# DanieleTeni/Online-Non-Linear-Centroidal-MPC-with-stability-Guarantees-for-Robust-Locomotion-of-Legged-Robots-

Measured on AMD Instinct MI355X. Metric: centroidal-MPC solves/sec, N=20 horizon, higher is better.
Workload: dtype f64

## Files before the change

### __graft_entry__.py

```python
import os
import sys

ROOT = os.path.dirname(os.path.abspath(__file__))
if ROOT not in sys.path:
    sys.path.insert(0, ROOT)


def build():
    import build as _b
    _b.build_hip()
    _b.build_oracle()
    _b.build_emu()
    _b.build_emu_gain()
    _b.build_emu_consts()
    _b.build_device_unit()
    _b.build_tools()
    import ctypes
    import torch
    import cmpc_amd
    from cmpc_amd import capi
    lib = ctypes.CDLL(capi.LIB_PATH)
    for sym in capi.SYMBOLS:
        getattr(lib, sym)


def smoke():
    import numpy as np
    import torch
    import cmpc_amd
    from cmpc_amd import workloads as wl
    from cmpc_amd.solver import BatchedCentroidalMPC
    from oracle import oracle_lib as ol

    assert torch.cuda.is_available(), "smoke() needs a GPU"
    spec, rec = wl.make_workload("perturbed", B=8, N=10, scale=0.25)
    solver = BatchedCentroidalMPC(spec, device="cuda:0")
    out, status, iters, kkt = solver.solve(torch.from_numpy(rec).to("cuda:0"))
# ... 18 lines not shown
```

### build.py

```python
import os
import subprocess
import sys

ROOT = os.path.dirname(os.path.abspath(__file__))
PKG = os.path.join(ROOT, "online-non-linear-centroidal-mpc-with-stability-guarantees-for-robust-locomotion-of-legged-robots-_amd")


def _newer(target, sources):
    if not os.path.exists(target):
        return True
    t = os.path.getmtime(target)
    return any(os.path.getmtime(s) > t for s in sources)


def build_hip(force=False, verbose=False):
    src = os.path.join(PKG, "csrc", "cmpc_hip.hip")
    wbc = os.path.join(PKG, "csrc", "wbc_qp.hip")
    deps = [src, wbc, os.path.join(PKG, "csrc", "cmpc_kernel.hpp"), os.path.join(PKG, "csrc", "cmpc_lds_asm.hpp"), os.path.join(PKG, "csrc", "cmpc_wave.hpp"), os.path.join(PKG, "csrc", "cmpc_order_fit.h"),
            os.path.join(ROOT, "include", "cmpc.h"), os.path.join(ROOT, "include", "cmpc_wbc.h")]
    out = os.path.join(PKG, "libcmpc_amd.so")
    if force or _newer(out, deps):
        cmd = ["hipcc", "--offload-arch=gfx950", "-O3", "-std=c++17", "-fPIC", "-shared", "-o", out, src, wbc]
        if verbose:
            cmd.insert(1, "-Rpass-analysis=kernel-resource-usage")
# ... 44 lines not shown

def build_emu_gain(force=False):
    src = os.path.join(ROOT, "tests", "emu", "cmpc_emu_gain.cpp")
    out = os.path.join(ROOT, "tests", "emu", "libcmpc_emu_gain.so")
    deps = [src, os.path.join(ROOT, "tests", "emu", "cmpc_emu.cpp"), os.path.join(PKG, "csrc", "cmpc_kernel.hpp"),
            os.path.join(PKG, "csrc", "cmpc_lds_asm.hpp"), os.path.join(PKG, "csrc", "cmpc_wave.hpp"),
            os.path.join(ROOT, "include", "cmpc.h")]
    if force or _newer(out, deps):
        subprocess.check_call(["g++", "-O2", "-std=c++17", "-mfma", "-ffp-contract=off", "-fPIC", "-shared", "-pthread", "-o", out, src])
    return out


def build_emu_consts(force=False):
    src = os.path.join(ROOT, "tests", "emu", "cmpc_emu_consts.cpp")
    out = os.path.join(ROOT, "tests", "emu", "libcmpc_emu_consts.so")
    deps = [src, os.path.join(ROOT, "tests", "emu", "cmpc_emu.cpp"), os.path.join(PKG, "csrc", "cmpc_kernel.hpp"),
            os.path.join(PKG, "csrc", "cmpc_lds_asm.hpp"), os.path.join(PKG, "csrc", "cmpc_wave.hpp"),
            os.path.join(ROOT, "include", "cmpc.h")]
    if force or _newer(out, deps):
        subprocess.check_call(["g++", "-O2", "-std=c++17", "-mfma", "-ffp-contract=off", "-fPIC", "-shared", "-pthread", "-o", out, src])
    return out


def build_device_unit(force=False):
    src = os.path.join(ROOT, "tests", "gpu_unit", "cmpc_device_unit.hip")
    out = os.path.join(ROOT, "tests", "gpu_unit", "libcmpc_device_unit.so")
    deps = [src, os.path.join(PKG, "csrc", "cmpc_kernel.hpp"), os.path.join(PKG, "csrc", "cmpc_lds_asm.hpp"), os.path.join(PKG, "csrc", "cmpc_wave.hpp")]
    if force or _newer(out, deps):
        subprocess.check_call(["hipcc", "--offload-arch=gfx950", "-O3", "-std=c++17", "-fPIC", "-shared", "-o", out, src])
    return out


def build_tools(force=False):
    outs = []
    for name in ("hbm_calib", "lds_b128_repro"):
        src = os.path.join(ROOT, "tools", "ubench", name + ".hip")
        out = os.path.join(ROOT, "tools", "ubench", name)
        if force or _newer(out, [src]):
            r = subprocess.run(["hipcc", "--offload-arch=gfx950", "-O3", "-o", out, src], capture_output=True, text=True)
            if r.returncode != 0:
                print(f"build_tools: {name} failed to compile (profiling scripts that need it will not run)\n{r.stderr}",
                      file=sys.stderr)
                continue
        outs.append(out)
    return outs


if __name__ == "__main__":
    force = "--force" in sys.argv
    print(build_hip(force, verbose="-v" in sys.argv))
    print(build_oracle(force))
    print(build_emu(force))
    print(build_emu_gain(force))
    print(build_emu_consts(force))
    print(build_device_unit(force))
    print(build_tools(force))
```

### online-non-linear-centroidal-mpc-with-stability-guarantees-for-robust-locomotion-of-legged-robots-_amd/csrc/cmpc_hip.hip

```cpp
#include <hip/hip_runtime.h>
#include <stdio.h>
#include <stdlib.h>
#include <string.h>
#include <string>

#include "cmpc_kernel.hpp"
#include "cmpc_order_fit.h"

#ifndef CMPC_WAVES_PER_SIMD
#define CMPC_WAVES_PER_SIMD 2
#endif

namespace {

constexpr int ORDER_BUCKETS = 64;
constexpr int ORDER_COUNTERS = 3 + 2 * ORDER_BUCKETS;

__device__ __forceinline__ int cmpc_order_bucket(const double *__restrict__ r, int N, double omega, double cz_max) {
  double gl = r[24 + 17], gr = r[24 + 18];
  const double gl0 = gl, gr0 = gr;
  int first = N, nsw = 0;
  double gain = 0.0;
  for (int k = 1; k <= N; ++k) {
    const double l = (k < N) ? r[24 + 19 * k + 17] : r[22], q = (k < N) ? r[24 + 19 * k + 18] : r[23];
// ... 391 lines not shown
  h->grid = h->num_cu * resident_per_cu(spec->nv);
  if (spec->nv == 4) {
    h->pair_per_cu = pairs_per_cu();
#ifdef CMPC_DEV_KNOBS
    if (const char *e = getenv("CMPC_PAIR_PER_CU")) { if (atoi(e) == 2 && h->pair_per_cu > 2) h->pair_per_cu = 2; }
#endif
    h->pair_grid = h->num_cu * h->pair_per_cu;
    h->pair_max_batch = (h->pair_per_cu >= 3 ? 14 : 8) * h->num_cu;
    if (spec->kernel == CMPC_KERNEL_SINGLE) h->pair_max_batch = 0;
    if (spec->kernel == CMPC_KERNEL_PAIR) h->pair_max_batch = 1 << 30;
#ifdef CMPC_DEV_KNOBS
    if (const char *e = getenv("CMPC_PAIR")) h->pair_max_batch = (atoi(e) == 0) ? 0 : 1 << 30;
#endif
  }
  h->slabs = slab_count(spec, h->num_cu);
#ifdef CMPC_DEV_KNOBS
  if (const char *e = getenv("CMPC_WG_PER_CU")) {
    const int n = atoi(e);
    if (n >= 1 && n < resident_per_cu(spec->nv)) h->grid = h->num_cu * n;
  }
#endif
  h->slab_doubles = slab_doubles(spec);
#ifdef CMPC_PROFILE
  if (hipMalloc(&h->prof, 28 * sizeof(long long)) == hipSuccess) (void)hipMemset(h->prof, 0, 28 * sizeof(long long));
#endif
  if (hipMalloc(&h->scratch, (size_t)h->slabs * h->slab_doubles * sizeof(double)) != hipSuccess ||
      hipMalloc(&h->ticket, ORDER_COUNTERS * sizeof(int)) != hipSuccess || hipEventCreate(&h->ev0) != hipSuccess ||
      hipEventCreate(&h->ev1) != hipSuccess) {
    cmpc_destroy(h);
    return fail(nullptr, "cmpc_create: device allocation failed");
  }
  *out = h;
  return 0;
}

int cmpc_destroy(cmpc_handle *h) {
  if (!h) return 0;
  DeviceGuard guard(h->device);
  if (h->scratch) (void)hipFree(h->scratch);
  if (h->ticket) (void)hipFree(h->ticket);
  if (h->order) (void)hipFree(h->order);
  if (h->gbuf) (void)hipFree(h->gbuf);
  if (h->ev0) (void)hipEventDestroy(h->ev0);
  if (h->ev1) (void)hipEventDestroy(h->ev1);
  delete h;
  return 0;
}
// ... 204 lines not shown
  const int blocks = B < 256 * 32 ? B : 256 * 32;
  hipLaunchKernelGGL(cmpc_build_records_kernel, dim3((unsigned)blocks), dim3(256), 0, (hipStream_t)stream, tb->T, N, rate,
                     B, nrec, t, state, tb->com_tab, tb->pose_l, tb->pose_r, tb->gl, tb->gr, tb->cur_l, tb->cur_r,
                     plan_pos, tb->n_steps, tb->slot_l, tb->slot_r, records);
  if (hipGetLastError() != hipSuccess) return fail(nullptr, "cmpc_build_records: launch failed");
  return 0;
}

const char *cmpc_last_kernel_name(cmpc_handle *h) { return h ? h->last_kernel : ""; }
const char *cmpc_last_error(cmpc_handle *h) { return h ? h->err.c_str() : g_err.c_str(); }
const char *cmpc_version(void) { return "cmpc_amd 0.5 (gfx950)"; }

#ifdef CMPC_DEV_KNOBS
int cmpc_debug_slab(cmpc_handle *h, double **ptr, size_t *doubles) {
  if (!h || !ptr || !doubles) return 1;
  *ptr = h->scratch; *doubles = h->slab_doubles;
  return 0;
}
#endif

#ifdef CMPC_PROFILE
int cmpc_profile_read(cmpc_handle *h, long long *out8) {
  if (!h || !h->prof) return 1;
  if (hipMemcpy(out8, h->prof, 28 * sizeof(long long), hipMemcpyDeviceToHost) != hipSuccess) return 1;
  (void)hipMemset(h->prof, 0, 28 * sizeof(long long));
  return 0;
}
#endif

}
```

### online-non-linear-centroidal-mpc-with-stability-guarantees-for-robust-locomotion-of-legged-robots-_amd/csrc/cmpc_kernel.hpp

```cpp
#pragma once
#include "../../include/cmpc.h"
#include <math.h>
#include <utility>
#ifdef CMPC_HOST_EMU
#include <cstdio>
#include <cstdlib>
#endif

#ifndef CMPC_HOST_EMU
#include <hip/hip_runtime.h>
#define CMPC_DEV __device__ __forceinline__
#define CMPC_LANE ((int)threadIdx.x)
#define CMPC_SYNC() asm volatile("s_waitcnt lgkmcnt(0)" ::: "memory")
#define CMPC_SYNC_GLOBAL() __syncthreads()
#define CMPC_SYNC_WG() asm volatile("s_waitcnt lgkmcnt(0)\n\ts_barrier" ::: "memory")
#define CMPC_WAVE_ID() ((int)__builtin_amdgcn_readfirstlane((int)threadIdx.x >> 6))
static __device__ __forceinline__ double cmpc_bcast(double v, int src) {
  union { double d; int i[2]; } u; u.d = v;
  u.i[0] = __builtin_amdgcn_readlane(u.i[0], src);
  u.i[1] = __builtin_amdgcn_readlane(u.i[1], src);
  return u.d;
}
#define CMPC_BCAST(v, src) cmpc_bcast((v), (src))
typedef double cmpc_v4d __attribute__((ext_vector_type(4)));
#define CMPC_MFMA_F64(a, b, c) __builtin_amdgcn_mfma_f64_16x16x4f64((a), (b), (c), 0, 0, 0)
#include "cmpc_wave.hpp"
#define CMPC_PAIR_OF(M, v, a, b) cmpc_pair_of<M>((v), (a), (b))
#define CMPC_OPAQUE(x) asm volatile("" : "+v"(x))
#define CMPC_OPAQUE_D(x) asm volatile("" : "+v"(x))
#define CMPC_UNIFORM_INT(x) __builtin_amdgcn_readfirstlane(x)
static __device__ __forceinline__ double cmpc_fresh(double a) { asm volatile("" : "+s"(a)); return a; }
#define CMPC_FRESH_D(x) cmpc_fresh(x)
#ifdef CMPC_FRESH_SPEC
#define SPD(field) cmpc_fresh(CMPC_SPEC_OR_ROW(field))
#else
#define SPD(field) CMPC_SPEC_OR_ROW(field)
#endif
typedef const double __attribute__((address_space(4))) *cmpc_crow_t;
#define CMPC_CROW(p) ((cmpc_crow_t)(p))
static __device__ __forceinline__ cmpc_crow_t cmpc_fresh_row(cmpc_crow_t r) { asm volatile("" : "+s"(r)); return r; }
#define CMPC_ROW_AT(r, i) (cmpc_fresh_row(r)[i])
static __device__ __forceinline__ double cmpc_uniform_d(double v) {
  union { double d; int i[2]; } u; u.d = v;
  int lo, hi;
  asm("s_nop 0\n\tv_readfirstlane_b32 %0, %2\n\tv_readfirstlane_b32 %1, %3\n\ts_nop 1" : "=s"(lo), "=s"(hi) : "v"(u.i[0]), "v"(u.i[1]));
  u.i[0] = lo; u.i[1] = hi;
  return u.d;
}
#ifdef CMPC_NO_UNIFORM_D
#define CMPC_UNIFORM_D(x) (x)
#else
#define CMPC_UNIFORM_D(x) cmpc_uniform_d(x)
#endif
#define CMPC_SCHED_FENCE() __builtin_amdgcn_sched_barrier(0)
#define CMPC_RELANE(x) do { (x) = (int)__builtin_amdgcn_mbcnt_hi(~0u, __builtin_amdgcn_mbcnt_lo(~0u, 0u)) + lane_base; } while (0)
#define CMPC_SYNC_WAVE(w) CMPC_SYNC()
#define CMPC_FENCE_WAVE(w) asm volatile("s_waitcnt vmcnt(0) lgkmcnt(0)" ::: "memory")
#endif
#ifdef CMPC_HOST_EMU
// ... 1 lines not shown
#define CMPC_FENCE_WAVE(w) emu_barrier_wait(&emu_wave_barrier[(w)])
#define CMPC_SYNC_WG() emu_barrier_wait(&emu_barrier)
#endif
#ifndef CMPC_RELANE
#define CMPC_RELANE(x) do { } while (0)
#define SPD(field) CMPC_SPEC_OR_ROW(field)
typedef const double *cmpc_crow_t;
#define CMPC_CROW(p) ((cmpc_crow_t)(p))
#define CMPC_ROW_AT(r, i) ((r)[i])
#define CMPC_FRESH_D(x) (x)
#define CMPC_UNIFORM_D(x) (x)
#endif
#define CMPC_CIDX(field) ((int)((__builtin_offsetof(cmpc_spec, field) - __builtin_offsetof(cmpc_spec, delta)) / sizeof(double)))
#define CMPC_SPEC_OR_ROW(field) (CONSTS ? CMPC_ROW_AT(crow, CMPC_CIDX(field)) : sp.field)
static_assert(CMPC_CIDX(relax) == CMPC_NCONST - 1 && CMPC_CIDX(box[2]) == 13 && __builtin_offsetof(cmpc_spec, tol) == __builtin_offsetof(cmpc_spec, relax) + sizeof(double),
              "the row of per-instance constants is the block of cmpc_spec from delta to relax");
#define CMPC_FMA(x, y, z) __builtin_fma((x), (y), (z))
#ifndef CMPC_OPAQUE_D
#define CMPC_OPAQUE_D(x) do { } while (0)
#endif
#ifndef CMPC_UNIFORM_INT
#define CMPC_UNIFORM_INT(x) (x)
#endif

#if defined(CMPC_PROFILE) && !defined(CMPC_HOST_EMU)
#define CMPC_TICK(slot) do { long long now_ = clock64(); tprof[slot] += now_ - tlast; tlast = now_; } while (0)
#define CMPC_TICK_RESET() do { tlast = clock64(); } while (0)
#else
#define CMPC_TICK(slot) do { } while (0)
#define CMPC_TICK_RESET() do { } while (0)
#endif

namespace cmpc {

struct KArgs {
  cmpc_spec sp;
  int B;
  const double *recs;
  const double *warm;
  const double *state_in;
  double *state_out;
  double *out;
  int32_t *status;
  int32_t *iters;
  double *kkt;
  double *scratch;
  size_t scratch_stride;
  long long *prof;
  double tol_acc, tol_tenth;
};

enum { R_LYAP = 0, R_CZ = 1, R_HWC = 2, R_BOX = 3, R_FRIC = 15 };

constexpr double ACC_FACTOR = 100.0;
// ... 154 lines not shown
  static_assert(3 * S::NF <= S::NZ, "r_j fits");
  static constexpr int LDS_DOUBLES = oEND + (oEND & 1);
};

template <int NV, int NW = 1, bool PIPE = false> struct Dims : LdsMap<NV, NW, PIPE> {
  using S = Sizes<NV, NW>;
  using Lm = LdsMap<NV, NW, PIPE>;
  static constexpr int WS = S::WS, NF = S::NF, NU = S::NU, NXA = S::NXA, NZ = S::NZ, NI = S::NI, NTRI = S::NTRI, NH = S::NH,
                       PS = S::PS, LS = S::LS, NPT = S::NPT;
  static constexpr bool COMPACT = (NV == 4 && NW == 1);
  static constexpr int gM = 0;
  static constexpr bool W_MERGE = (NZ <= WS);
  static constexpr int gAL = ((NTRI + 7) / 8) * 8;
  static constexpr int gGH = gAL + NZ;
  static constexpr int GHS = WS * NH;
  static constexpr int gB = gGH + 3 * GHS;
  static constexpr int gPB = gB + NXA;
  static constexpr int gPV = gPB + NXA;
  static constexpr int gL = gPV + NXA;
  static constexpr int gG = gL + NU;
  static constexpr int gL1 = gG + NI;
  static constexpr int gPV1 = gL1 + NU;
  static constexpr int STAGE = ((gPV1 + NXA + 7) / 8) * 8;
  static constexpr int state_lam(int N) { return CMPC_NSOL(N, NV); }
  static constexpr int state_s(int N) { return state_lam(N) + (N + 1) * NXA; }
  static constexpr int state_z(int N) { return state_s(N) + (N + 1) * NI; }
  static constexpr int state_mu(int N) { return state_z(N) + (N + 1) * NI; }
  static constexpr int state_fl(int N) { return state_mu(N) + 8; }
  static_assert(state_fl(20) + 2 * 21 == CMPC_NSTATE(20, NV), "layout of include/cmpc.h");
  static size_t scratch_doubles(int N) {
    size_t n = (size_t)(N + 1) * STAGE;
    n += (size_t)(N + 1) * NXA * 4;
    n += (size_t)(N + 1) * NU * 3;
    n += (size_t)(N + 1) * NI * 4;
    return (n + 7) / 8 * 8;
  }
};

#ifndef CMPC_NO_DEVICE_CODE

CMPC_DEV int tri(int i) { return i * (i + 1) / 2; }

typedef double cmpc_v2d __attribute__((vector_size(16)));
struct GArr {
  double *p;
  CMPC_DEV double &operator[](unsigned i) const { return *(double *)((char *)p + (size_t)(i * 8u)); }
  CMPC_DEV cmpc_v2d &pair(unsigned i) const { return *(cmpc_v2d *)((char *)p + (size_t)(i * 16u)); }
};

CMPC_DEV bool consts_row_ok(cmpc_crow_t row) {
  bool ok = true;
  for (int i = 0; i < CMPC_NCONST; ++i) {
    const double v = row[i];
    const bool positive = i == CMPC_CIDX(delta) || i == CMPC_CIDX(g) || (i >= CMPC_CIDX(cz_max) && i <= CMPC_CIDX(foot_width));
    const bool gain = i == CMPC_CIDX(k1) || i == CMPC_CIDX(k2);
    ok = ok && v < INFINITY && v > -INFINITY && (positive ? v > 0.0 : (gain || v >= 0.0));
  }
  return ok;
}

template <int NV, int NW = 1, bool PIPE = false, bool GAIN = false, bool CONSTS = false> struct Solver {
  using D = Dims<NV, NW, PIPE>;
  static constexpr int XCH_DU = 16, XCH_DOUBLES = XCH_DU + 2 * D::NU;
  static_assert(!PIPE || XCH_DOUBLES <= D::P_DOUBLES, "the exchange words fit in the unused P region of the second image");
  static constexpr int XCH_AT = D::LDS_DOUBLES + D::oP;
  static_assert(!PIPE || NW == 1, "the pipelined pair runs the one-wave solver");
  static_assert(!PIPE || (D::oUB + 64 <= D::oBV && D::oUB >= D::oXN1 + D::NXA && !D::GT_FIRST),
                "pair_vectors reads BV / writes XN1 of the image the Riccati wave is working in");
  static constexpr int NF = D::NF, NU = D::NU, NXA = D::NXA, NZ = D::NZ, NI = D::NI, NH = D::NH, WS = D::WS;
  static_assert(NW == 1 || NU <= 64, "the input rows (pivot chains, substitutions) live in the first wave");

  const KArgs &ka;
  const cmpc_spec &sp;
  double *lds;
  double *ldsR;
  int lane_base = 0;
  GArr gs;
  GArr rec;
  int N, lane;
  int wv = 0;
  GArr gx, glam, gdx, glamn, gu, gdu, gupx, gsl, gz, gds, gdz;
  int lr[NH][6];
  double lg[NH][6];
  double piv_min = PIV_MIN;
  GArr st_in{nullptr};
  long long tprof[28] = {0, 0, 0, 0, 0, 0, 0, 0, 0, 0, 0, 0, 0, 0, 0, 0, 0, 0, 0, 0, 0, 0, 0, 0, 0, 0, 0, 0}, tlast = 0;
  double *gain_out = nullptr;
  GArr gbuf{nullptr};
  bool gain_sweep = false;
  cmpc_crow_t crow = nullptr;

  CMPC_DEV Solver(const KArgs &a, double *l, double *g, const double *r)
      : ka(a), sp(a.sp), lds(l), ldsR(l), gs{g}, rec{const_cast<double *>(r)}, N(a.sp.N), lane(CMPC_LANE) {
    if constexpr (NW > 1 || PIPE) wv = CMPC_WAVE_ID();
    if constexpr (NW > 1) lane_base = 64 * wv;
    if constexpr (PIPE) lane &= 63;
    if constexpr (NW == 1 && !PIPE) CMPC_RELANE(lane);
    double *p = g + (size_t)(N + 1) * D::STAGE;
    gx = GArr{p}; p += (size_t)(N + 1) * NXA;
    glam = GArr{p}; p += (size_t)(N + 1) * NXA;
    gdx = GArr{p}; p += (size_t)(N + 1) * NXA;
    glamn = GArr{p}; p += (size_t)(N + 1) * NXA;
    gu = GArr{p}; p += (size_t)(N + 1) * NU;
    gdu = GArr{p}; p += (size_t)(N + 1) * NU;
    gupx = GArr{p}; p += (size_t)(N + 1) * NU;
    gsl = GArr{p}; p += (size_t)(N + 1) * NI;
    gz = GArr{p}; p += (size_t)(N + 1) * NI;
    gds = GArr{p}; p += (size_t)(N + 1) * NI;
    gdz = GArr{p};
  }
  CMPC_DEV GArr stage(int k) const { return GArr{gs.p + (size_t)k * D::STAGE}; }
  CMPC_DEV double &L(int o) const { return lds[o]; }
  CMPC_DEV double &R(int o) const { return ldsR[o]; }
  CMPC_DEV void image(int k) { if constexpr (PIPE) lds = ldsR + (k & 1) * D::LDS_DOUBLES; }
  CMPC_DEV void sync() const {
    if constexpr (PIPE) { CMPC_SYNC_WAVE(wv); }
    else {
#ifdef CMPC_HOST_EMU
      CMPC_SYNC();
#else
      if constexpr (NW == 1) CMPC_SYNC(); else CMPC_SYNC_WG();
#endif
    }
  }
  CMPC_DEV void gsync() const {
    if constexpr (PIPE) { CMPC_FENCE_WAVE(wv); } else { CMPC_SYNC_GLOBAL(); }
  }
  CMPC_DEV void pair_sync() const { if constexpr (PIPE) { CMPC_SYNC_GLOBAL(); } }
  CMPC_DEV bool first_wave() const { return NW == 1 || wv == 0; }

  CMPC_DEV double gam_k(int k, int f) const { return (k == N) ? L(D::oHDR + 22 + f) : L(D::oSR + 17 + f); }
  CMPC_DEV double gam_km1(int f) const { return L(D::oSRP + 17 + f); }
  CMPC_DEV void vert_local(int j, double &vx, double &vy) const {
    const double Lh = SPD(foot_length) * 0.5, Wh = SPD(foot_width) * 0.5;
// ... 944 lines not shown
        for (int q = 0; q < NXA; q += 4) {
          b0 += pr[q] * bv[q]; b1 += pr[q + 1] * bv[q + 1]; b2 += pr[q + 2] * bv[q + 2]; b3 += pr[q + 3] * bv[q + 3];
        }
      } else {
        const double *pr = &R(D::oP + lane * D::PS);
#pragma unroll
        for (int q = 0; q < NXA; q += 4) {
          b0 += pr[q] * bv[q]; b1 += pr[q + 1] * bv[q + 1]; b2 += pr[q + 2] * bv[q + 2]; b3 += pr[q + 3] * bv[q + 3];
        }
      }
      const double a = (b0 + b1) + (b2 + b3);
      L(D::oXN1 + lane) = R(D::oPC + lane) + a;
      st[D::gB + lane] = L(D::oBV + lane);
    }
  }
  CMPC_DEV double list_dot(int h, const double *v) const {
    double a = 0.0;
#pragma unroll
    for (int n = 0; n < 6; ++n) a = CMPC_FMA(lg[h][n], v[lr[h][n]], a);
    CMPC_OPAQUE_D(a);
    return a;
  }

  CMPC_DEV void eval_stage(int k, double mu, double reg, double wz, double x0n2, Err &er, bool init) {
    CMPC_RELANE(lane); CMPC_OPAQUE(lane);
    load_stage(k);
    CMPC_TICK(24);
    const GArr st = stage(k);
    if (k < N) {
      stage_geometry(k);
    } else {
      for (int c = lane; c < 3 * NZ; c += WS) L(D::oGH + c) = 0.0;
      if (lane < NXA) L(D::oBV + lane) = 0.0;
      sync();
    }
    CMPC_TICK(11);
    double gl_dot[NH];
    if constexpr (D::GT_FIRST) {
      if (k < N && lane < NXA) er.e_p = fmax(er.e_p, fabs(L(D::oBV + lane)));
      build_list(&L(D::oGH), (k < N) ? L(D::oSR + 17) : 0.0, (k < N) ? L(D::oSR + 18) : 0.0, L(D::oHDR + 20));
      if (lane < NZ) { st[D::gGH + lane] = lg[0][1]; st[D::gGH + D::GHS + lane] = lg[0][2]; st[D::gGH + 2 * D::GHS + lane] = lg[0][3]; }
      if (k < N) {
        form_Pb(st);
        sync();
        CMPC_TICK(13);
        gl_dot[0] = list_dot(0, &L(D::oLAMN));
        if (lane < NZ) { L(D::oH0 + lane) = list_dot(0, &L(D::oXN1)); L(D::oH1 + lane) = list_dot(0, &R(D::oPC1)); }
        gt_phase<false>(L(D::oSR + 17), L(D::oSR + 18), L(D::oHDR + 20));
      } else {
        gl_dot[0] = 0.0;
        for (int e = lane; e < D::NTRI; e += WS) L(D::oM + e) = 0.0;
        sync();
      }
      CMPC_RELANE(lane); CMPC_OPAQUE(lane);
    }
    stage_ineq(k, x0n2);
    CMPC_TICK(12);
    for (int r = lane; r < NI; r += WS) {
      const bool act = L(D::oW2 + r) != 0.0;
      const double g = L(D::oGK + r);
      double s = L(D::oSK + r), z = L(D::oZK + r);
      if (init) {
        const bool carry = act && s > 0.0 && z > 0.0;
        s = carry ? s : (act ? fmax(-g, fmin(1e-2, sqrt(mu))) : 1.0);
        z = carry ? z : (act ? mu / s : 0.0);
        L(D::oZK + r) = z;
        gsl[k * NI + r] = s; gz[k * NI + r] = z;
      }
      if (act) {
        double sg = z / s;
        if constexpr (GAIN) { if (gain_sweep) sg = fmin(sg, (r >= R_BOX && r < R_FRIC) ? GAIN_SIG_CAP_BOX : GAIN_SIG_CAP); }
        L(D::oW0 + r) = sg; L(D::oW1 + r) = sg * (g + s); L(D::oW2 + r) = 1.0 / s;
        er.e_p = fmax(er.e_p, fabs(g + s));
        er.e_c = fmax(er.e_c, fabs(s * z)); er.e_cmu = fmax(er.e_cmu, fabs(s * z - mu));
        er.sum_mult += fabs(z); er.n_mult += 1;
      } else {
        L(D::oW0 + r) = 0.0; L(D::oW1 + r) = 0.0; L(D::oW2 + r) = 0.0; L(D::oZK + r) = 0.0;
      }
// ... 9 lines not shown
      CMPC_RELANE(lane); CMPC_OPAQUE(lane);
      build_list(&L(D::oGH), (k < N) ? L(D::oSR + 17) : 0.0, (k < N) ? L(D::oSR + 18) : 0.0, L(D::oHDR + 20));
    }
#pragma unroll
    for (int h = 0; h < NH; ++h) {
      const int col = lane + WS * h;
      if (col >= NZ) continue;
      const double ho = cost_grad(k, col, wz);
      double jw[3];
      jgt3(k, col, jw);
      double r = ho + jw[0];
      if constexpr (D::GT) {
        if constexpr (!D::GT_FIRST) gl_dot[h] = (k < N) ? list_dot(h, &L(D::oLAMN)) : 0.0;
        r += gl_dot[h];
      } else {
        if (k < N) for (int n = 0; n < 6; ++n) r += lg[h][n] * L(D::oLAMN + lr[h][n]);
      }
      if (col >= NU) r -= L(D::oLAMK + col - NU);
      const bool is_var = (col < NU) ? (k < N) : (k >= 1);
      if (is_var) er.e_d = fmax(er.e_d, fabs(r));
      double h0 = ho + jw[1] + mu * jw[2];
      double h1 = jw[2];
      CMPC_OPAQUE_D(h0); CMPC_OPAQUE_D(h1);
      if constexpr (D::GT_FIRST) {
        if (k < N) { L(D::oH0 + col) = h0 + L(D::oH0 + col); L(D::oH1 + col) = h1 + L(D::oH1 + col); }
        else { L(D::oH0 + col) = h0; L(D::oH1 + col) = h1; }
      } else {
        L(D::oH0 + col) = h0; L(D::oH1 + col) = h1;
      }
      st[D::gAL + col] = L(D::oAL + col);
    }
    CMPC_TICK(26);
    if constexpr (!D::GT_FIRST) {
#pragma unroll
      for (int h = 0; h < NH; ++h) {
        const int c = lane + WS * h;
        if (c < NZ) { st[D::gGH + c] = L(D::oGH + c); st[D::gGH + D::GHS + c] = L(D::oGH + NZ + c); st[D::gGH + 2 * D::GHS + c] = L(D::oGH + 2 * NZ + c); }
      }
    }
    for (int r = lane; r < NI; r += WS) st[D::gG + r] = L(D::oGK + r);
    CMPC_TICK(0);
    if constexpr (D::GT_FIRST) {
      CMPC_RELANE(lane); CMPC_OPAQUE(lane);
      build_H(k, reg, wz);
      CMPC_TICK(1);
    }
    sync();
  }
  CMPC_DEV bool riccati_stage(int k) {
    const GArr st = stage(k);
    if constexpr (PIPE) {
      CMPC_RELANE(lane); CMPC_OPAQUE(lane);
      build_list(&L(D::oGH), (k < N) ? L(D::oSR + 17) : 0.0, (k < N) ? L(D::oSR + 18) : 0.0, L(D::oHDR + 20));
    }
    if (k < N) {
      if constexpr (!D::GT_FIRST) {
        if constexpr (!PIPE) form_Pb(st);
        sync();
        CMPC_TICK(13);
        CMPC_RELANE(lane); CMPC_OPAQUE(lane);
        gt_phase<true>(L(D::oSR + 17), L(D::oSR + 18), L(D::oHDR + 20));
        CMPC_TICK(14);
      }
      CMPC_RELANE(lane); CMPC_OPAQUE(lane);
// ... 48 lines not shown
            cmpc_lds_word pa[14];
            double v[14];
#pragma unroll
            for (int q = 0; q < 14; ++q) {
              const cmpc_lds_word alt = wc + CMPC_LDS_WORDS(tri(NU + q0 + q) + NU - (q0 + q));
              pa[q] = (wt > alt) ? wt : alt;
            }
            if (q0 == 0) lds_read_gather_off14<0>(v, pa); else lds_read_gather_off14<14>(v, pa);
#pragma unroll
            for (int q = 0; q < 14; ++q) pr[q0 + q] = v[q];
          }
        }
#pragma unroll
        for (int q = 0; q < NXA; q += 4) {
          b0 += pr[q] * bv[q]; b1 += pr[q + 1] * bv[q + 1]; b2 += pr[q + 2] * bv[q + 2]; b3 += pr[q + 3] * bv[q + 3];
        }
        other[D::oXN1 + lane] = (b0 + b1) + (b2 + b3);
        stage(k - 1)[D::gB + lane] = bv[lane];
      }
    }
    sync();
  }

  CMPC_DEV bool matrix_sweep(double mu, double reg, double x0n2, Err &er, bool init) {
    er.e_d = er.e_p = er.e_c = er.e_cmu = er.sum_mult = 0.0; er.n_mult = 0;
    piv_min = fmax(PIV_MIN, PIV_FRAC * reg);
    const double e1 = 2.718281828459045235360287;
    double ez = CMPC_UNIFORM_D(exp(-(double)(N - 1)));
    CMPC_OPAQUE_D(ez);
    if constexpr (!PIPE) {
      for (int k = N; k >= 0; --k) {
        const double wz = SPD(w_cz_const) * 0.5 * ez + SPD(w_cz_const) * 0.5;
        ez *= e1;
        eval_stage(k, mu, reg, wz, x0n2, er, init);
        if (!riccati_stage(k)) return false;
      }
      return true;
    } else {
      double *xch = ldsR + XCH_AT;
      if (lane == 0 && wv == 0) { xch[8] = 0.0; xch[9] = 0.0; }
      CMPC_SYNC_WG();
      for (int j = 0; j <= N + 2; ++j) {
        if (wv == 1) {
          const int kv = N - j + 2, k = N - j;
          if (kv >= 0 && kv <= N) { image(kv); pair_vectors(kv); }
          const double wz = SPD(w_cz_const) * 0.5 * ez + SPD(w_cz_const) * 0.5;
          ez *= e1;
          if (k >= 0) { image(k); eval_stage(k, mu, reg, wz, x0n2, er, init); }
        } else if (j >= 1 && j <= N + 1) {
          const int k = N - j + 1;
          image(k);
          if (!riccati_stage(k) && lane == 0) xch[8 + (j & 1)] = 1.0;
        }
        CMPC_SYNC_WG();
        const bool failed = xch[8 + (j & 1)] != 0.0;
        if (failed) { image(0); CMPC_SYNC_WG(); return false; }
      }
      image(0);
// ... 550 lines not shown
        for (int c = 0; c < G; ++c) { const double du = CMPC_BCAST(y[c], cu); acc[c] += cf * du; }
      } else {
        const int sx = col - NU;
        if (sx < G) acc[sx] += cf;
      }
    }
    if (lane < CMPC_NX) {
#pragma unroll
      for (int c = 0; c < G; ++c) gout[lane * G + c] = acc[c];
    }
  }

  CMPC_DEV void gain_tail(int st, bool saved, const double *warm) {
    const bool usable = st == CMPC_CONVERGED || st == CMPC_ACCEPTABLE;
    bool good = false;
    if (usable) {
      if (saved) {
        st_in = gbuf;
        if (!PIPE || wv == 0) initial_point(gbuf.p, warm, true);
        if constexpr (PIPE) pair_sync(); else gsync();
      }
      Err er;
      gain_sweep = true;
      good = matrix_sweep(sp.tol, 0.0, 0.0, er, false);
      if constexpr (PIPE) pair_sync(); else gsync();
    }
    if (wv == 0) gain_step(good);
    if constexpr (PIPE) pair_sync(); else gsync();
  }

  CMPC_DEV void reject(double *state_out, double *out_, int32_t *status, int32_t *iters, double *kkt_out) {
    if (!PIPE || wv == 0) {
      const GArr out{out_};
      const double nanv = __builtin_nan("");
      for (int e = lane; e < (N + 1) * CMPC_NX + N * NU; e += WS) out[e] = nanv;
      if (lane == 0) {
        *status = CMPC_NUMERICAL; *iters = 0; *kkt_out = INFINITY;
        if (state_out) { GArr{state_out}[D::state_mu(N)] = 0.0; GArr{state_out}[D::state_mu(N) + 1] = 0.0; }
      }
    }
    if constexpr (PIPE) pair_sync(); else sync();
  }

  CMPC_DEV void solve(const double *warm, const double *state_in, double *state_out, double *out, int32_t *status,
                      int32_t *iters, double *kkt_out) {
    auto tol_ = [&]() { return CMPC_FRESH_D(sp.tol); };
    const double tol_acc = ka.tol_acc, tol_10 = ka.tol_tenth;
    const double x0n2 = 0.0;
    bool resume = false;
    if (state_in) {
      const double ms = GArr{const_cast<double *>(state_in)}[D::state_mu(N)];
      resume = ms > 0.0 && ms < INFINITY;
      if (resume) st_in = GArr{const_cast<double *>(state_in)};
    }
    int st = CMPC_MAX_ITER, it = 0, spent = 0;
    bool ret_saved = false;
    double kkt = INFINITY;
    for (;;) {
    if (state_out && lane == 0) GArr{state_out}[D::state_mu(N)] = 0.0;
    double mu = resume ? st_in[D::state_mu(N)] : MU_INIT;
    kkt = INFINITY; st = CMPC_MAX_ITER;
    constexpr bool CNT_LDS = (NW == 1);
    int n_acc = 0, n_stall = 0, polish = -1, since_best = 0;
    constexpr int SAVED = 256;
    constexpr int NOSTEP = 512;
    double &reg_last = R(D::oCOLD + 0), &kkt_best = R(D::oCOLD + 1), &kkt_saved = R(D::oCOLD + 2);
    double &snapped = R(D::oCOLD + 3);
    {
      double inf = INFINITY, zero = 0.0;
      CMPC_OPAQUE_D(inf); CMPC_OPAQUE_D(zero);
      const double ks0 = kkt_saved;
      if constexpr (PIPE) { CMPC_SYNC_WG(); } else sync();
      double at0 = sp.acc_tol;
      CMPC_OPAQUE_D(at0);
      const bool carry = spent > 0 && ks0 <= fmax(at0, tol_());
      reg_last = zero; kkt_best = inf; snapped = zero;
      if (!carry) kkt_saved = inf;
      if constexpr (CNT_LDS) { R(D::oCOLD + 4) = zero; R(D::oCOLD + 5) = zero; R(D::oCOLD + 6) = zero - 1.0; R(D::oCOLD + 7) = zero; }
    }
    auto acc_raw = [&]() { double a = sp.acc_tol; CMPC_OPAQUE_D(a); return a; };
    auto acc_tol = [&]() { return fmax(acc_raw(), tol_()); };
    auto save_tol = [&]() { return fmax(fmax(acc_raw(), tol_()), tol_acc); };
    if (!PIPE || wv == 0) initial_point(resume ? state_in : warm, warm, resume);
    pair_sync();
    CMPC_TICK_RESET();
    for (it = 0; it <= sp.max_iter - spent; ++it) {
      double reg = 0.0;
      Err er;
      bool fail = false;
      const double mu_sweep = mu;
      const double rl = reg_last;
#ifdef CMPC_TEST_FAIL_ITER
      if (!resume && it == (CMPC_TEST_FAIL_ITER)) fail = true; else
#endif
      while (!matrix_sweep(mu, reg, x0n2, er, it == 0)) {
        sync();
        if (reg == 0.0) reg = (rl == 0.0) ? 1e-4 : fmax(1e-20, rl / 3);
        else reg *= (rl == 0.0) ? 100.0 : 8.0;
        if (reg > 1e20) { fail = true; break; }
      }
      if (fail) { st = CMPC_NUMERICAL | NOSTEP; break; }
#ifdef CMPC_DEBUG_FIRST_SWEEP
      if (it == 0) break;
#endif
      double e_d = red_max(er.e_d), e_p = red_max(er.e_p), e_c = red_max(er.e_c), e_cmu = red_max(er.e_cmu);
      double sm = red_sum(er.sum_mult), nm = red_sum((double)er.n_mult);
      if constexpr (PIPE) {
        double *xch = ldsR + XCH_AT;
        if (wv == 1 && lane == 0) { xch[0] = e_d; xch[1] = e_p; xch[2] = e_c; xch[3] = e_cmu; xch[4] = sm; xch[5] = nm; }
        pair_sync();
        e_d = xch[0]; e_p = xch[1]; e_c = xch[2]; e_cmu = xch[3]; sm = xch[4]; nm = xch[5];
      }
      const double sd = fmax(100.0, sm / fmax(nm, 1.0)) / 100.0;
      kkt = fmax(fmax(e_d / sd, e_p), e_c / sd);
#ifdef CMPC_HOST_EMU
      if (lane == 0 && getenv("CMPC_EMU_TRACE"))
        printf("it %3d d=%.2e p=%.2e c=%.2e mu=%.1e reg=%.1e\n", it, e_d / sd, e_p, e_c / sd, mu, reg);
#endif
      const double ebar = fmax(fmax(e_d / sd, e_p), e_cmu / sd);
// ... 78 lines not shown
      }
    }
    bool use_saved = (st & SAVED) != 0;
    const bool nostep = (st & NOSTEP) != 0;
    st &= SAVED - 1;
    const double ks_end = kkt_saved;
    if (nostep && ks_end <= acc_tol()) { st = CMPC_ACCEPTABLE; kkt = ks_end; use_saved = true; }
    const bool keep = resume && (st == CMPC_MAX_ITER || st == CMPC_NUMERICAL) && ks_end <= acc_tol();
    if (keep && !(it < sp.max_iter)) { st = CMPC_ACCEPTABLE; kkt = ks_end; use_saved = true; }
    if (!use_saved && !keep && (!PIPE || wv == 0)) write_solution(out);
    if constexpr (GAIN) ret_saved = use_saved;
    const int again = CMPC_UNIFORM_INT((int)(resume && (st == CMPC_MAX_ITER || st == CMPC_NUMERICAL) && it < sp.max_iter));
    if (!again) break;
    spent = CMPC_UNIFORM_INT(spent + it); resume = false;
    if constexpr (PIPE) pair_sync(); else gsync();
    }
    if (lane == 0 && (!PIPE || wv == 0)) {
      *status = st; *iters = it + spent; *kkt_out = kkt;
      if (state_out) GArr{state_out}[D::state_mu(N) + 1] = (double)(it + spent);
    }
    if constexpr (GAIN) gain_tail(st, ret_saved, warm);
#if defined(CMPC_PROFILE) && !defined(CMPC_HOST_EMU)
    if (lane == 0 && ka.prof)
      for (int i = 0; i < 28; ++i) atomicAdd((unsigned long long *)&ka.prof[i], (unsigned long long)tprof[i]);
#endif
    if constexpr (PIPE) pair_sync(); else sync();
  }
};

#endif
}
```

Baseline: 88490.

## Reuse stage evaluations across regularization retries of the Riccati sweep

When the Riccati factorization fails and the sweep is retried with larger regularization, stages already processed in the failed sweep now reload parked Hessian terms, inequality weights and geometry from an extra per-stage scratch area instead of re-running the stage geometry and inequality evaluation. The accumulated error measures are parked in LDS so that retries start from them. This adds global scratch writes on every non-initial sweep, more scratch memory, a stronger barrier between retries and possible register pressure, in exchange for cheaper retries. It only applies to the single-wave, non-pipelined, non-gain configuration.

```diff
diff --git a/__graft_entry__.py b/__graft_entry__.py
--- a/__graft_entry__.py
+++ b/__graft_entry__.py
@@ -13,6 +13,8 @@
     _b.build_emu()
     _b.build_emu_gain()
     _b.build_emu_consts()
+    _b.build_emu_reuse()
+    _b.build_emu_reuse(reuse=False)
     _b.build_device_unit()
     _b.build_tools()
     import ctypes
diff --git a/build.py b/build.py
--- a/build.py
+++ b/build.py
@@ -90,6 +90,29 @@
     return out
 
 
+def build_emu_reuse(force=False, reuse=True):
+    src = os.path.join(ROOT, "tests", "emu", "cmpc_emu_reuse.cpp")
+    out = os.path.join(ROOT, "tests", "emu", "libcmpc_emu_reuse.so" if reuse else "libcmpc_emu_noreuse.so")
+    deps = [src, os.path.join(ROOT, "tests", "emu", "cmpc_emu.cpp"), os.path.join(PKG, "csrc", "cmpc_kernel.hpp"),
+            os.path.join(PKG, "csrc", "cmpc_lds_asm.hpp"), os.path.join(PKG, "csrc", "cmpc_wave.hpp"),
+            os.path.join(ROOT, "include", "cmpc.h")]
+    if force or _newer(out, deps):
+        subprocess.check_call(["g++", "-O2", "-std=c++17", "-mfma", "-ffp-contract=off", "-fPIC", "-shared", "-pthread"]
+                              + ([] if reuse else ["-DCMPC_NO_EVAL_REUSE"]) + ["-o", out, src])
+    return out
+
+
+def build_hip_no_reuse(force=False, profile=False):
+    src = os.path.join(PKG, "csrc", "cmpc_hip.hip")
+    deps = [src, os.path.join(PKG, "csrc", "cmpc_kernel.hpp"), os.path.join(PKG, "csrc", "cmpc_lds_asm.hpp"), os.path.join(PKG, "csrc", "cmpc_wave.hpp"),
+            os.path.join(ROOT, "include", "cmpc.h")]
+    out = os.path.join(ROOT, "tools", "libcmpc_amd_noreuse_prof.so" if profile else "libcmpc_amd_noreuse.so")
+    if force or _newer(out, deps):
+        subprocess.check_call(["hipcc", "--offload-arch=gfx950", "-O3", "-std=c++17", "-fPIC", "-shared", "-DCMPC_NO_EVAL_REUSE"]
+                              + (["-DCMPC_PROFILE"] if profile else []) + ["-o", out, src, os.path.join(PKG, "csrc", "wbc_qp.hip")])
+    return out
+
+
 def build_device_unit(force=False):
     src = os.path.join(ROOT, "tests", "gpu_unit", "cmpc_device_unit.hip")
     out = os.path.join(ROOT, "tests", "gpu_unit", "libcmpc_device_unit.so")
@@ -121,5 +144,7 @@
     print(build_emu(force))
     print(build_emu_gain(force))
     print(build_emu_consts(force))
+    print(build_emu_reuse(force))
+    print(build_emu_reuse(force, reuse=False))
     print(build_device_unit(force))
     print(build_tools(force))
diff --git a/online-non-linear-centroidal-mpc-with-stability-guarantees-for-robust-locomotion-of-legged-robots-_amd/csrc/cmpc_hip.hip b/online-non-linear-centroidal-mpc-with-stability-guarantees-for-robust-locomotion-of-legged-robots-_amd/csrc/cmpc_hip.hip
--- a/online-non-linear-centroidal-mpc-with-stability-guarantees-for-robust-locomotion-of-legged-robots-_amd/csrc/cmpc_hip.hip
+++ b/online-non-linear-centroidal-mpc-with-stability-guarantees-for-robust-locomotion-of-legged-robots-_amd/csrc/cmpc_hip.hip
@@ -437,7 +437,7 @@
 #endif
   h->slab_doubles = slab_doubles(spec);
 #ifdef CMPC_PROFILE
-  if (hipMalloc(&h->prof, 28 * sizeof(long long)) == hipSuccess) (void)hipMemset(h->prof, 0, 28 * sizeof(long long));
+  if (hipMalloc(&h->prof, CMPC_NPROF * sizeof(long long)) == hipSuccess) (void)hipMemset(h->prof, 0, CMPC_NPROF * sizeof(long long));
 #endif
   if (hipMalloc(&h->scratch, (size_t)h->slabs * h->slab_doubles * sizeof(double)) != hipSuccess ||
       hipMalloc(&h->ticket, ORDER_COUNTERS * sizeof(int)) != hipSuccess || hipEventCreate(&h->ev0) != hipSuccess ||
@@ -688,10 +688,10 @@
 #ifdef CMPC_PROFILE
 int cmpc_profile_read(cmpc_handle *h, long long *out8) {
   if (!h || !h->prof) return 1;
-  if (hipMemcpy(out8, h->prof, 28 * sizeof(long long), hipMemcpyDeviceToHost) != hipSuccess) return 1;
-  (void)hipMemset(h->prof, 0, 28 * sizeof(long long));
-  return 0;
-}
-#endif
-
-}
+  if (hipMemcpy(out8, h->prof, CMPC_NPROF * sizeof(long long), hipMemcpyDeviceToHost) != hipSuccess) return 1;
+  (void)hipMemset(h->prof, 0, CMPC_NPROF * sizeof(long long));
+  return 0;
+}
+#endif
+
+}
diff --git a/online-non-linear-centroidal-mpc-with-stability-guarantees-for-robust-locomotion-of-legged-robots-_amd/csrc/cmpc_kernel.hpp b/online-non-linear-centroidal-mpc-with-stability-guarantees-for-robust-locomotion-of-legged-robots-_amd/csrc/cmpc_kernel.hpp
--- a/online-non-linear-centroidal-mpc-with-stability-guarantees-for-robust-locomotion-of-legged-robots-_amd/csrc/cmpc_kernel.hpp
+++ b/online-non-linear-centroidal-mpc-with-stability-guarantees-for-robust-locomotion-of-legged-robots-_amd/csrc/cmpc_kernel.hpp
@@ -28,13 +28,14 @@
 #define CMPC_PAIR_OF(M, v, a, b) cmpc_pair_of<M>((v), (a), (b))
 #define CMPC_OPAQUE(x) asm volatile("" : "+v"(x))
 #define CMPC_OPAQUE_D(x) asm volatile("" : "+v"(x))
+#define CMPC_OPAQUE_S(x) asm volatile("" : "+s"(x))
 #define CMPC_UNIFORM_INT(x) __builtin_amdgcn_readfirstlane(x)
 static __device__ __forceinline__ double cmpc_fresh(double a) { asm volatile("" : "+s"(a)); return a; }
 #define CMPC_FRESH_D(x) cmpc_fresh(x)
 #ifdef CMPC_FRESH_SPEC
 #define SPD(field) cmpc_fresh(CMPC_SPEC_OR_ROW(field))
 #else
-#define SPD(field) CMPC_SPEC_OR_ROW(field)
+#define SPD(field) (EVAL_REUSE ? cmpc_fresh(CMPC_SPEC_OR_ROW(field)) : CMPC_SPEC_OR_ROW(field))
 #endif
 typedef const double __attribute__((address_space(4))) *cmpc_crow_t;
 #define CMPC_CROW(p) ((cmpc_crow_t)(p))
@@ -82,14 +83,34 @@
 #ifndef CMPC_UNIFORM_INT
 #define CMPC_UNIFORM_INT(x) (x)
 #endif
+#ifndef CMPC_OPAQUE_S
+#define CMPC_OPAQUE_S(x) do { } while (0)
+#endif
 
 #if defined(CMPC_PROFILE) && !defined(CMPC_HOST_EMU)
-#define CMPC_TICK(slot) do { long long now_ = clock64(); tprof[slot] += now_ - tlast; tlast = now_; } while (0)
+static __device__ __forceinline__ constexpr int cmpc_retry_class(int slot) {
+  return (slot == 11 || slot == 12 || slot == 26 || slot == 0) ? 31
+       : (slot == 24 || slot == 25) ? 32
+       : (slot == 27) ? 34
+       : 33;
+}
+#define CMPC_TICK(slot) do { long long now_ = clock64(); tprof[slot] += now_ - tlast; \
+    if (prof_retry) tprof[cmpc_retry_class(slot)] += now_ - tlast; \
+    tlast = now_; } while (0)
 #define CMPC_TICK_RESET() do { tlast = clock64(); } while (0)
+#define CMPC_RETRY_STAT(slot, n) do { tprof[slot] += (n); } while (0)
+#define CMPC_RETRY_MARK(on) do { prof_retry = (on); } while (0)
+#define CMPC_RETRY_TRACK 1
 #else
 #define CMPC_TICK(slot) do { } while (0)
 #define CMPC_TICK_RESET() do { } while (0)
-#endif
+#define CMPC_RETRY_MARK(on) do { } while (0)
+#define CMPC_RETRY_TRACK 0
+#endif
+#ifndef CMPC_RETRY_STAT
+#define CMPC_RETRY_STAT(slot, n) do { } while (0)
+#endif
+#define CMPC_NPROF 36
 
 namespace cmpc {
 
@@ -290,6 +311,8 @@
   static constexpr int gL1 = gG + NI;
   static constexpr int gPV1 = gL1 + NU;
   static constexpr int STAGE = ((gPV1 + NXA + 7) / 8) * 8;
+  static constexpr int rH0 = 0, rH1 = rH0 + NZ, rW0 = rH1 + NZ, rVDV = rW0 + NI, rQ = rVDV + 3 * NF, rPI = rQ + 2;
+  static constexpr int RE_STAGE = COMPACT ? ((rPI + 3 + 7) / 8) * 8 : 0;
   static constexpr int state_lam(int N) { return CMPC_NSOL(N, NV); }
   static constexpr int state_s(int N) { return state_lam(N) + (N + 1) * NXA; }
   static constexpr int state_z(int N) { return state_s(N) + (N + 1) * NI; }
@@ -301,6 +324,7 @@
     n += (size_t)(N + 1) * NXA * 4;
     n += (size_t)(N + 1) * NU * 3;
     n += (size_t)(N + 1) * NI * 4;
+    n += (size_t)(N + 1) * RE_STAGE;
     return (n + 7) / 8 * 8;
   }
 };
@@ -337,6 +361,15 @@
                 "pair_vectors reads BV / writes XN1 of the image the Riccati wave is working in");
   static constexpr int NF = D::NF, NU = D::NU, NXA = D::NXA, NZ = D::NZ, NI = D::NI, NH = D::NH, WS = D::WS;
   static_assert(NW == 1 || NU <= 64, "the input rows (pivot chains, substitutions) live in the first wave");
+#ifdef CMPC_NO_EVAL_REUSE
+  static constexpr bool EVAL_REUSE = false;
+#else
+  static constexpr bool EVAL_REUSE = NV == 4 && NW == 1 && !PIPE && !GAIN && D::GT_FIRST;
+#endif
+  static constexpr bool RETRY_TRACK_POSSIBLE = NV == 4 && NW == 1 && !PIPE && !GAIN;
+  static constexpr int ER_AT = 256;
+  static_assert(!RETRY_TRACK_POSSIBLE || (ER_AT >= 3 * NZ + NXA + 3 * NF && ER_AT + 6 * WS <= D::NTRI), "the parked error measures fit the M region");
+  static constexpr bool RETRY_TRACK = EVAL_REUSE || (CMPC_RETRY_TRACK && NV == 4 && NW == 1 && !PIPE && !GAIN);
 
   const KArgs &ka;
   const cmpc_spec &sp;
@@ -352,7 +385,8 @@
   double lg[NH][6];
   double piv_min = PIV_MIN;
   GArr st_in{nullptr};
-  long long tprof[28] = {0, 0, 0, 0, 0, 0, 0, 0, 0, 0, 0, 0, 0, 0, 0, 0, 0, 0, 0, 0, 0, 0, 0, 0, 0, 0, 0, 0}, tlast = 0;
+  long long tprof[CMPC_NPROF] = {0, 0, 0, 0, 0, 0, 0, 0, 0, 0, 0, 0, 0, 0, 0, 0, 0, 0, 0, 0, 0, 0, 0, 0, 0, 0, 0, 0, 0, 0, 0, 0, 0, 0, 0, 0}, tlast = 0;
+  bool prof_retry = false;
   double *gain_out = nullptr;
   GArr gbuf{nullptr};
   bool gain_sweep = false;
@@ -378,6 +412,10 @@
     gdz = GArr{p};
   }
   CMPC_DEV GArr stage(int k) const { return GArr{gs.p + (size_t)k * D::STAGE}; }
+  CMPC_DEV unsigned restage(int k) const {
+    CMPC_OPAQUE_S(k);
+    return (unsigned)((N + 1 - k) * D::STAGE + (N + 1) * (4 * NXA + 3 * NU + 4 * NI) + k * D::RE_STAGE);
+  }
   CMPC_DEV double &L(int o) const { return lds[o]; }
   CMPC_DEV double &R(int o) const { return ldsR[o]; }
   CMPC_DEV void image(int k) { if constexpr (PIPE) lds = ldsR + (k & 1) * D::LDS_DOUBLES; }
@@ -1368,12 +1406,39 @@
     return a;
   }
 
-  CMPC_DEV void eval_stage(int k, double mu, double reg, double wz, double x0n2, Err &er, bool init) {
+  CMPC_DEV void eval_stage(int k, double mu, double reg, double wz, double x0n2, Err &er, bool init, bool reuse_ = false) {
+    const bool reuse = EVAL_REUSE && reuse_;
     CMPC_RELANE(lane); CMPC_OPAQUE(lane);
+    if constexpr (EVAL_REUSE) { CMPC_OPAQUE_S(k); }
+    double re_h0 = 0.0, re_h1 = 0.0, re_al = 0.0, re_w0 = 0.0;
+    if (reuse) {
+      const GArr sk = stage(k); const unsigned re = restage(k);
+      const int cz = (lane < NZ) ? lane : 0, ci = (lane < NI) ? lane : 0;
+      re_al = sk[D::gAL + cz]; re_w0 = sk[re + D::rW0 + ci]; re_h0 = sk[re + D::rH0 + cz]; re_h1 = sk[re + D::rH1 + cz];
+    }
     load_stage(k);
     CMPC_TICK(24);
     const GArr st = stage(k);
-    if (k < N) {
+    if (reuse) {
+      const unsigned re = restage(k);
+      const int cz = (lane < NZ) ? lane : 0, cx = (lane < NXA) ? lane : 0, ci = (lane < NI) ? lane : 0;
+      static_assert(!EVAL_REUSE || (NH == 1 && NI <= WS && 3 * NF + 5 <= WS && D::rQ == D::rVDV + 3 * NF && D::rPI == D::rQ + 2), "one word of each kept vector per lane");
+      const double re_gh0 = st[D::gGH + cz], re_gh1 = st[D::gGH + D::GHS + cz], re_gh2 = st[D::gGH + 2 * D::GHS + cz];
+      const double re_bv = st[D::gB + cx];
+      const double re_vdv = st[re + D::rVDV + ((lane < 3 * NF + 5) ? lane : 0)];
+      const int dump = D::oDUMP + (lane & (D::DUMPN - 1));
+      const bool in_z = lane < NZ;
+      L(in_z ? D::oGH + lane : dump) = re_gh0; L(in_z ? D::oGH + NZ + lane : dump) = re_gh1; L(in_z ? D::oGH + 2 * NZ + lane : dump) = re_gh2;
+      L((lane < NXA) ? D::oBV + lane : dump) = (k < N) ? re_bv : 0.0;
+      L((lane < 3 * NF) ? D::oVDV + lane : (lane < 3 * NF + 2) ? D::oMISC + 30 - 3 * NF + lane
+        : (lane < 3 * NF + 5) ? D::oMISC + 9 - (3 * NF + 2) + lane : dump) = re_vdv;
+      static_assert(!EVAL_REUSE || (D::oLAMK == D::oUK + NU && NU + NXA == NZ), "the Lyapunov gradient fits the inputs and lam_k");
+      L(in_z ? D::oUK + lane : dump) = re_al; L(in_z ? D::oH0 + lane : dump) = re_h0; L(in_z ? D::oH1 + lane : dump) = re_h1;
+      L((lane < NI) ? D::oSK + lane : dump) = re_w0;
+      sync();
+      CMPC_RETRY_STAT(30, 1);
+      CMPC_TICK(27);
+    } else if (k < N) {
       stage_geometry(k);
     } else {
       for (int c = lane; c < 3 * NZ; c += WS) L(D::oGH + c) = 0.0;
@@ -1391,7 +1456,10 @@
         sync();
         CMPC_TICK(13);
         gl_dot[0] = list_dot(0, &L(D::oLAMN));
-        if (lane < NZ) { L(D::oH0 + lane) = list_dot(0, &L(D::oXN1)); L(D::oH1 + lane) = list_dot(0, &R(D::oPC1)); }
+        if (lane < NZ) {
+          const double a0 = list_dot(0, &L(D::oXN1)), a1 = list_dot(0, &R(D::oPC1));
+          L(D::oH0 + lane) = reuse ? L(D::oH0 + lane) + a0 : a0; L(D::oH1 + lane) = reuse ? L(D::oH1 + lane) + a1 : a1;
+        }
         gt_phase<false>(L(D::oSR + 17), L(D::oSR + 18), L(D::oHDR + 20));
       } else {
         gl_dot[0] = 0.0;
@@ -1400,6 +1468,12 @@
       }
       CMPC_RELANE(lane); CMPC_OPAQUE(lane);
     }
+    if (reuse) {
+      const int dump = D::oDUMP + (lane & (D::DUMPN - 1));
+      const double al_ = L(D::oUK + ((lane < NZ) ? lane : 0)), w0_ = L(D::oSK + ((lane < NI) ? lane : 0));
+      L((lane < NZ) ? D::oAL + lane : dump) = al_; L((lane < NI) ? D::oW0 + lane : dump) = w0_;
+      sync();
+    } else {
     stage_ineq(k, x0n2);
     CMPC_TICK(12);
     for (int r = lane; r < NI; r += WS) {
@@ -1455,6 +1529,7 @@
       double h0 = ho + jw[1] + mu * jw[2];
       double h1 = jw[2];
       CMPC_OPAQUE_D(h0); CMPC_OPAQUE_D(h1);
+      if constexpr (EVAL_REUSE) { if (!init) { const unsigned re = restage(k); st[re + D::rH0 + col] = h0; st[re + D::rH1 + col] = h1; } }
       if constexpr (D::GT_FIRST) {
         if (k < N) { L(D::oH0 + col) = h0 + L(D::oH0 + col); L(D::oH1 + col) = h1 + L(D::oH1 + col); }
         else { L(D::oH0 + col) = h0; L(D::oH1 + col) = h1; }
@@ -1472,7 +1547,17 @@
       }
     }
     for (int r = lane; r < NI; r += WS) st[D::gG + r] = L(D::oGK + r);
+    if constexpr (EVAL_REUSE) {
+      if (!init) {
+        const unsigned re = restage(k);
+        if (lane < NI) st[re + D::rW0 + lane] = L(D::oW0 + lane);
+        if (lane < 3 * NF) st[re + D::rVDV + lane] = L(D::oVDV + lane);
+        if (lane < 2) st[re + D::rQ + lane] = L(D::oMISC + 30 + lane);
+        if (lane < 3) st[re + D::rPI + lane] = L(D::oMISC + 9 + lane);
+      }
+    }
     CMPC_TICK(0);
+    }
     if constexpr (D::GT_FIRST) {
       CMPC_RELANE(lane); CMPC_OPAQUE(lane);
       build_H(k, reg, wz);
@@ -1567,8 +1652,14 @@
     sync();
   }
 
-  CMPC_DEV bool matrix_sweep(double mu, double reg, double x0n2, Err &er, bool init) {
+  CMPC_DEV bool matrix_sweep(double mu, double reg, double x0n2, Err &er, bool init, int &k_done) {
+    const bool retry = RETRY_TRACK && k_done <= N;
     er.e_d = er.e_p = er.e_c = er.e_cmu = er.sum_mult = 0.0; er.n_mult = 0;
+    if (retry) {
+      const double *w = &L(D::oM + ER_AT + 6 * lane);
+      er.e_d = w[0]; er.e_p = w[1]; er.e_c = w[2]; er.e_cmu = w[3]; er.sum_mult = w[4]; er.n_mult = (int)w[5];
+      CMPC_RETRY_STAT(28, 1);
+    }
     piv_min = fmax(PIV_MIN, PIV_FRAC * reg);
     const double e1 = 2.718281828459045235360287;
     double ez = CMPC_UNIFORM_D(exp(-(double)(N - 1)));
@@ -1577,8 +1668,26 @@
       for (int k = N; k >= 0; --k) {
         const double wz = SPD(w_cz_const) * 0.5 * ez + SPD(w_cz_const) * 0.5;
         ez *= e1;
-        eval_stage(k, mu, reg, wz, x0n2, er, init);
-        if (!riccati_stage(k)) return false;
+        if constexpr (RETRY_TRACK) {
+          const bool done = k >= k_done;
+          CMPC_RETRY_MARK(done);
+          if (EVAL_REUSE || !done) eval_stage(k, mu, reg, wz, x0n2, er, init, done);
+          else { Err again = er; eval_stage(k, mu, reg, wz, x0n2, again, init); }
+          if (!riccati_stage(k)) {
+            CMPC_RETRY_MARK(false);
+            if (!init) { CMPC_RETRY_STAT(29, N + 1 - k); if (k < k_done) k_done = CMPC_UNIFORM_INT(k); }
+            if (retry) CMPC_RETRY_STAT(35, 1);
+            if (!init) {
+              double *w = &L(D::oM + ER_AT + 6 * lane);
+              w[0] = er.e_d; w[1] = er.e_p; w[2] = er.e_c; w[3] = er.e_cmu; w[4] = er.sum_mult; w[5] = (double)er.n_mult;
+            }
+            return false;
+          }
+          CMPC_RETRY_MARK(false);
+        } else {
+          eval_stage(k, mu, reg, wz, x0n2, er, init);
+          if (!riccati_stage(k)) return false;
+        }
       }
       return true;
     } else {
@@ -2175,7 +2284,8 @@
       }
       Err er;
       gain_sweep = true;
-      good = matrix_sweep(sp.tol, 0.0, 0.0, er, false);
+      int k_done = N + 1;
+      good = matrix_sweep(sp.tol, 0.0, 0.0, er, false, k_done);
       if constexpr (PIPE) pair_sync(); else gsync();
     }
     if (wv == 0) gain_step(good);
@@ -2197,6 +2307,9 @@
 
   CMPC_DEV void solve(const double *warm, const double *state_in, double *state_out, double *out, int32_t *status,
                       int32_t *iters, double *kkt_out) {
+#if !defined(CMPC_HOST_EMU)
+    if constexpr (EVAL_REUSE && !CONSTS) asm volatile("" ::: "v255");
+#endif
     auto tol_ = [&]() { return CMPC_FRESH_D(sp.tol); };
     const double tol_acc = ka.tol_acc, tol_10 = ka.tol_tenth;
     const double x0n2 = 0.0;
@@ -2243,11 +2356,12 @@
       bool fail = false;
       const double mu_sweep = mu;
       const double rl = reg_last;
+      int k_done = N + 1;
 #ifdef CMPC_TEST_FAIL_ITER
       if (!resume && it == (CMPC_TEST_FAIL_ITER)) fail = true; else
 #endif
-      while (!matrix_sweep(mu, reg, x0n2, er, it == 0)) {
-        sync();
+      while (!matrix_sweep(mu, reg, x0n2, er, it == 0, k_done)) {
+        if constexpr (EVAL_REUSE) gsync(); else sync();
         if (reg == 0.0) reg = (rl == 0.0) ? 1e-4 : fmax(1e-20, rl / 3);
         else reg *= (rl == 0.0) ? 100.0 : 8.0;
         if (reg > 1e20) { fail = true; break; }
@@ -2372,7 +2486,7 @@
     if constexpr (GAIN) gain_tail(st, ret_saved, warm);
 #if defined(CMPC_PROFILE) && !defined(CMPC_HOST_EMU)
     if (lane == 0 && ka.prof)
-      for (int i = 0; i < 28; ++i) atomicAdd((unsigned long long *)&ka.prof[i], (unsigned long long)tprof[i]);
+      for (int i = 0; i < CMPC_NPROF; ++i) atomicAdd((unsigned long long *)&ka.prof[i], (unsigned long long)tprof[i]);
 #endif
     if constexpr (PIPE) pair_sync(); else sync();
   }
```

New measurement: 90770 (median of 6 runs). +2.6%, better.
